# openshmem-org/openshmem-async

Hardware: AMD Instinct MI355X
Metric: GiB/s device-resident shmem_double_sum_to_all, nreduce=32Mi, 1/2/4/8 GPUs (higher is better)
Workload: dtype f64; 1 GPU; local reduce (fold acc = acc + in) of shmem_double_sum_to_all, 1 PE; nreduce=33554432, type=double, op=sum, PE_size=1, algo=fold, parallelism=one PE per GPU x1, transport=none (one PE: the step is the local fold, no exchange), arrays=symmetric heap (shmem_malloc, HBM)

## Files before the change

openshmem-async_amd/csrc/fold_kernels.hip:

```cpp
#include <hip/hip_ext.h>

#include <algorithm>
#include <atomic>
#include <mutex>
#include <vector>

#include "fold_ops.h"

namespace shmx {

enum KernelKind { kKindFold = 0, kKindCopy = 1, kKindPeers = 2, kKindGather = 3, kKindOrders = 4 };
namespace {
constexpr size_t kClockPairs = 4096;
struct KClock {
    std::mutex mu;
    std::atomic<bool> on{false};
    std::vector<hipEvent_t> ev;
    std::vector<int> kind;
    size_t used = 0;
    size_t dropped = 0;
} g_kclock;

bool clock_pair(int kind, hipEvent_t *a, hipEvent_t *b) {
    if (!g_kclock.on.load(std::memory_order_relaxed)) return false;
    std::lock_guard<std::mutex> lk(g_kclock.mu);
    if (g_kclock.used >= kClockPairs) {
        ++g_kclock.dropped;
        return false;
    }
    if (g_kclock.ev.size() < 2 * (g_kclock.used + 1)) {
// ... 67 lines not shown
    size_t nvec;
    size_t tail;
    int peers;
    unsigned long long *sig_word;
    unsigned long long sig_value;
    void *out2;
};

__device__ __forceinline__ void signal_host_done(const FoldArgs &args) {
    if (!args.sig_word) return;
    asm volatile("s_waitcnt vmcnt(0)" ::: "memory");
    __syncthreads();
    if (threadIdx.x == 0)
        __hip_atomic_store(args.sig_word, args.sig_value, __ATOMIC_RELEASE, __HIP_MEMORY_SCOPE_SYSTEM);
}


template <typename T, int OP, int NIN, int UNROLL, int NT>
__device__ __forceinline__ void fold_body(const FoldArgs &args) {
    constexpr int E = 16 / sizeof(T);
    const int nins = NIN > 0 ? NIN : args.nins;
    const size_t tid = (size_t)blockIdx.x * kBlock + threadIdx.x;
    const size_t nthr = (size_t)gridDim.x * kBlock;

    {
        T *out = static_cast<T *>(args.out);
        const size_t body_end = args.head + args.nvec * E;
        const size_t nscalar = args.head + args.tail;
        for (size_t s = tid; s < nscalar; s += nthr) {
            const size_t i = s < args.head ? s : body_end + (s - args.head);
            T acc = static_cast<const T *>(args.ins[0])[i];
            for (int k = 1; k < nins; ++k)
                acc = Op<T, OP>::ap(acc, static_cast<const T *>(args.ins[k])[i]);
            out[i] = acc;
            if constexpr (NIN == 1)
                if (args.out2) static_cast<T *>(args.out2)[i] = acc;
        }
    }
    if (args.nvec == 0) return;

    u32x4 *out = reinterpret_cast<u32x4 *>(static_cast<T *>(args.out) + args.head);
    u32x4 *out2 = NIN == 1 && args.out2 ? reinterpret_cast<u32x4 *>(static_cast<T *>(args.out2) + args.head)
                                        : nullptr;
    const size_t nvec = args.nvec;
    const size_t step = (size_t)gridDim.x * kBlock * UNROLL;
    for (size_t base = (size_t)blockIdx.x * kBlock * UNROLL; base < nvec;
// ... 31 lines not shown
                    u32x4 nxt[UNROLL];
#pragma unroll
                    for (int u = 0; u < UNROLL; ++u) nxt[u] = ld16<NT>(in_k(k) + v0 + u * kBlock);
#pragma unroll
                    for (int u = 0; u < UNROLL; ++u) {
                        acc[u] = apply16<T, OP>(acc[u], cur[u]);
                        cur[u] = nxt[u];
                    }
                }
#pragma unroll
                for (int u = 0; u < UNROLL; ++u) acc[u] = apply16<T, OP>(acc[u], cur[u]);
            } else {
                for (int k = 1; k < nins; ++k) {
                    const u32x4 *ink = reinterpret_cast<const u32x4 *>(
                        static_cast<const T *>(args.ins[k]) + args.head);
                    u32x4 x[UNROLL];
#pragma unroll
                    for (int u = 0; u < UNROLL; ++u) x[u] = ld16<NT>(ink + v0 + u * kBlock);
#pragma unroll
                    for (int u = 0; u < UNROLL; ++u) acc[u] = apply16<T, OP>(acc[u], x[u]);
                }
            }
#pragma unroll
            for (int u = 0; u < UNROLL; ++u) st16<NT>(out + v0 + u * kBlock, acc[u]);
            if constexpr (NIN == 1)
                if (out2)
#pragma unroll
                    for (int u = 0; u < UNROLL; ++u) st16<NT>(out2 + v0 + u * kBlock, acc[u]);
        } else {
            for (int u = 0; u < UNROLL; ++u) {
                const size_t v = v0 + (size_t)u * kBlock;
                if (v >= nvec) break;
                u32x4 acc = ld16<NT>(reinterpret_cast<const u32x4 *>(
                                         static_cast<const T *>(args.ins[0]) + args.head) + v);
                for (int k = 1; k < nins; ++k)
                    acc = apply16<T, OP>(acc, ld16<NT>(reinterpret_cast<const u32x4 *>(
                                                 static_cast<const T *>(args.ins[k]) + args.head) + v));
                st16<NT>(out + v, acc);
                if constexpr (NIN == 1)
                    if (out2) st16<NT>(out2 + v, acc);
            }
        }
    }
}

template <typename T, int OP, int NIN, int UNROLL, int NT>
__global__ __launch_bounds__(kBlock) void fold_kernel(FoldArgs args) {
    fold_body<T, OP, NIN, UNROLL, NT>(args);
    signal_host_done(args);
}

constexpr int kUnrollN = 4;
constexpr int kUnrollFold2 = 4;

constexpr int peers_unroll(int maxin) { return maxin <= 8 ? 4 : 2; }

template <typename T, int OP, int MAXIN, int NT>
__global__ __launch_bounds__(kBlock) void fold_peers_kernel(FoldArgs args) {
    constexpr int E = 16 / sizeof(T);
    constexpr int U = peers_unroll(MAXIN);
    const int nins = args.nins;
    const size_t tid = (size_t)blockIdx.x * kBlock + threadIdx.x;
    const size_t nthr = (size_t)gridDim.x * kBlock;
// ... 10 lines not shown
    }
    if (args.nvec == 0) return;
    auto in = [&](int k) {
        return reinterpret_cast<const u32x4 *>(static_cast<const T *>(args.ins[k]) + args.head);
    };
    u32x4 *out = reinterpret_cast<u32x4 *>(static_cast<T *>(args.out) + args.head);
    const size_t nvec = args.nvec;
    const size_t step = (size_t)gridDim.x * kBlock * U;
    for (size_t base = (size_t)blockIdx.x * kBlock * U; base < nvec; base += step) {
        const size_t v0 = base + threadIdx.x;
        if (base + (size_t)kBlock * U <= nvec) {
            u32x4 x[MAXIN][U];
#pragma unroll
            for (int k = 0; k < MAXIN; ++k)
                if (k < nins)
#pragma unroll
                    for (int u = 0; u < U; ++u) x[k][u] = ld16<NT>(in(k) + v0 + u * kBlock);
#pragma unroll
            for (int u = 0; u < U; ++u) {
                u32x4 acc = x[0][u];
#pragma unroll
                for (int k = 1; k < MAXIN; ++k)
                    if (k < nins) acc = apply16<T, OP>(acc, x[k][u]);
                st16<NT>(out + v0 + u * kBlock, acc);
            }
        } else {
            for (int u = 0; u < U; ++u) {
                const size_t v = v0 + (size_t)u * kBlock;
                if (v >= nvec) break;
                u32x4 acc = ld16<NT>(in(0) + v);
                for (int k = 1; k < nins; ++k) acc = apply16<T, OP>(acc, ld16<NT>(in(k) + v));
                st16<NT>(out + v, acc);
            }
        }
    }
}

constexpr int kUnrollOrders = 1;

struct OrdersArgs {
    void *outs[kMaxFoldInputs];
    const void *ins[kMaxFoldInputs];
    int nins;
    size_t head, nvec, tail;
};

template <typename T, int OP, int MAXIN, bool ROLLED, typename V, typename Ap, typename St>
__device__ __forceinline__ void fold_orders_of(const V (&x)[MAXIN], int nins, Ap ap, St store) {
    if constexpr (ROLLED) {
#pragma unroll 1
        for (int k = 0; k < nins; ++k) {
            V acc = x[0];
#pragma unroll
            for (int j = 1; j < MAXIN; ++j)
                if (j == k) acc = x[j];
// ... 29 lines not shown
        for (size_t s = tid; s < nscalar; s += nthr) {
            const size_t i = s < args.head ? s : body_end + (s - args.head);
            T x[MAXIN];
#pragma unroll
            for (int k = 0; k < MAXIN; ++k)
                if (k < nins) x[k] = static_cast<const T *>(args.ins[k])[i];
            fold_orders_of<T, OP, MAXIN, ROLLED>(
                x, nins, [](T a, T b) { return Op<T, OP>::ap(a, b); },
                [&](int k, T r) { static_cast<T *>(args.outs[k])[i] = r; });
        }
    }
    if (args.nvec == 0) return;
    auto in = [&](int k) {
        return reinterpret_cast<const u32x4 *>(static_cast<const T *>(args.ins[k]) + args.head);
    };
    auto out = [&](int k) { return reinterpret_cast<u32x4 *>(static_cast<T *>(args.outs[k]) + args.head); };
    auto ap16 = [](u32x4 a, u32x4 b) { return apply16<T, OP>(a, b); };
    const size_t nvec = args.nvec;
    for (size_t v = tid; v < nvec; v += nthr) {
        u32x4 x[MAXIN];
#pragma unroll
        for (int k = 0; k < MAXIN; ++k)
            if (k < nins) x[k] = ld16<NT>(in(k) + v);
        fold_orders_of<T, OP, MAXIN, ROLLED>(x, nins, ap16, [&](int k, u32x4 r) { st16<NT>(out(k) + v, r); });
    }
}


static size_t grid_for(const FoldArgs &a, int unroll) {
    size_t work_blocks;
    if (a.nvec > 0)
        work_blocks = (a.nvec + (size_t)kBlock * unroll - 1) / ((size_t)kBlock * unroll);
    else
        work_blocks = (a.head + a.tail + kBlock - 1) / kBlock;
    const size_t cap = a.nvec == 0 ? 2048 : (size_t)1 << 30;
    size_t blocks = work_blocks < cap ? work_blocks : cap;
    if (blocks < 1) blocks = 1;
    if (blocks > (size_t)INT_MAX) blocks = INT_MAX;
    return blocks;
}

hipError_t enqueue_marker(unsigned long long *word, unsigned long long value, hipStream_t stream) {
    return hipStreamWriteValue64(stream, word, value, 0);
}

template <typename T, int OP, int NT>
hipError_t launch_typed_grid(const FoldArgs &a, hipStream_t stream);
// ... 98 lines not shown
    case SHMEMX_OP_SUM: return launch_nt<T, SHMEMX_OP_SUM>(a, s);
    case SHMEMX_OP_PROD: return launch_nt<T, SHMEMX_OP_PROD>(a, s);
    default: return hipErrorInvalidValue;
    }
}

}

size_t type_size(int type) {
    switch (type) {
    case SHMEMX_TYPE_SHORT: return sizeof(short);
    case SHMEMX_TYPE_INT: return sizeof(int);
    case SHMEMX_TYPE_LONG: return sizeof(long);
    case SHMEMX_TYPE_LONGLONG: return sizeof(long long);
    case SHMEMX_TYPE_FLOAT: return sizeof(float);
    case SHMEMX_TYPE_DOUBLE: return sizeof(double);
    case SHMEMX_TYPE_LONGDOUBLE: return sizeof(long double);
    case SHMEMX_TYPE_COMPLEXD: return 2 * sizeof(double);
    case SHMEMX_TYPE_COMPLEXF: return 2 * sizeof(float);
    default: return 0;
    }
}

bool op_valid(int type, int op) {
    if (type < 0 || type >= SHMEMX_NTYPES || op < 0 || op >= SHMEMX_NOPS) return false;
    switch (op) {
    case SHMEMX_OP_SUM:
    case SHMEMX_OP_PROD: return true;
    case SHMEMX_OP_AND:
    case SHMEMX_OP_OR:
    case SHMEMX_OP_XOR: return type <= SHMEMX_TYPE_LONGLONG;
    default: return type != SHMEMX_TYPE_COMPLEXD && type != SHMEMX_TYPE_COMPLEXF;
    }
}

bool op_on_device(int type, int op) { return op_valid(type, op); }

namespace {

hipError_t dispatch(int type, int op, FoldArgs &a, const void *const *ptrs, int nptrs, size_t n,
                    hipStream_t stream) {
    const size_t sz = type_size(type);
    const uintptr_t off = reinterpret_cast<uintptr_t>(ptrs[0]) & 15u;
    bool same = (off % sz) == 0;
    for (int k = 1; k < nptrs && same; ++k)
        same = (reinterpret_cast<uintptr_t>(ptrs[k]) & 15u) == off;
    if (same) {
        size_t head = ((16 - off) & 15u) / sz;
        if (head > n) head = n;
        const size_t E = 16 / sz;
        a.head = head;
        a.nvec = (n - head) / E;
        a.tail = n - head - a.nvec * E;
    } else {
        a.head = n;
        a.nvec = 0;
        a.tail = 0;
    }
    if (a.nins == 1) {
        switch (sz) {
        case 2: return launch_copy<short>(a, stream);
        case 4: return launch_copy<int>(a, stream);
        case 8: return launch_copy<long>(a, stream);
        case 16: return launch_copy<cplxd>(a, stream);
        default: return hipErrorInvalidValue;
        }
    }
    switch (type) {
    case SHMEMX_TYPE_SHORT: return launch_int_ops<short>(op, a, stream);
    case SHMEMX_TYPE_INT: return launch_int_ops<int>(op, a, stream);
    case SHMEMX_TYPE_LONG:
    case SHMEMX_TYPE_LONGLONG: return launch_int_ops<long>(op, a, stream);
    case SHMEMX_TYPE_FLOAT: return launch_fp_ops<float>(op, a, stream);
    case SHMEMX_TYPE_DOUBLE: return launch_fp_ops<double>(op, a, stream);
    case SHMEMX_TYPE_LONGDOUBLE: return launch_fp_ops<ld80>(op, a, stream);
    case SHMEMX_TYPE_COMPLEXD: return launch_cplx_ops<cplxd>(op, a, stream);
    case SHMEMX_TYPE_COMPLEXF: return launch_cplx_ops<cplxf>(op, a, stream);
    default: return hipErrorInvalidValue;
    }
}

}

hipError_t launch_fold(int type, int op, void *out, const void *const *ins,
                       int nins, size_t n, hipStream_t stream) {
    if (!op_on_device(type, op) || nins < 1 || nins > kMaxFoldInputs || !out)
        return hipErrorInvalidValue;
    if (n == 0) return hipSuccess;
    FoldArgs a{};
    a.out = out;
    a.nins = nins;
    const void *ptrs[kMaxFoldInputs + 1];
    ptrs[0] = out;
    for (int k = 0; k < nins; ++k) {
        if (!ins[k]) return hipErrorInvalidValue;
        a.ins[k] = ins[k];
        ptrs[k + 1] = ins[k];
    }
    return dispatch(type, op, a, ptrs, nins + 1, n, stream);
}

bool copy_one_workgroup(int type, const void *dst, const void *src, size_t n) {
    const size_t sz = type_size(type);
    if (!sz || !n) return false;
    const uintptr_t off = reinterpret_cast<uintptr_t>(dst) & 15u;
    if (off % sz != 0 || (reinterpret_cast<uintptr_t>(src) & 15u) != off)
        return n <= (size_t)kBlock;
    size_t head = ((16 - off) & 15u) / sz;
    if (head > n) head = n;
    const size_t E = 16 / sz, nvec = (n - head) / E, tail = n - head - nvec * E;
    if (nvec == 0) return head + tail <= (size_t)kBlock;
    return nvec <= (size_t)kBlock * kUnrollCopy;
}

hipError_t launch_fold_signal(int type, int op, void *out, const void *const *ins, int nins, size_t n,
                              hipStream_t stream, const HostSignal &sig) {
    if (!op_on_device(type, op) || nins < 1 || nins > kMaxFoldInputs || !out || !sig.word)
        return hipErrorInvalidValue;
    if (n == 0) return launch_host_signal(sig, stream);
    FoldArgs a{};
    a.out = out;
    a.nins = nins;
    a.sig_word = sig.word;
    a.sig_value = sig.value;
    const void *ptrs[kMaxFoldInputs + 1];
    ptrs[0] = out;
    for (int k = 0; k < nins; ++k) {
        if (!ins[k]) return hipErrorInvalidValue;
        a.ins[k] = ins[k];
        ptrs[k + 1] = ins[k];
    }
    return dispatch(type, op, a, ptrs, nins + 1, n, stream);
}

hipError_t launch_copy2_signal(int type, void *out, void *out2, const void *in, size_t n, hipStream_t stream,
                               const HostSignal &sig) {
    if (!op_on_device(type, SHMEMX_OP_SUM) || !out || !out2 || !in || !sig.word) return hipErrorInvalidValue;
    if (n == 0) return launch_host_signal(sig, stream);
    FoldArgs a{};
    a.out = out;
    a.out2 = out2;
    a.nins = 1;
    a.ins[0] = in;
    a.sig_word = sig.word;
    a.sig_value = sig.value;
    const void *ptrs[3] = {out, out2, in};
    return dispatch(type, SHMEMX_OP_SUM, a, ptrs, 3, n, stream);
}

hipError_t launch_host_signal(const HostSignal &sig, hipStream_t stream) {
    if (!sig.word) return hipErrorInvalidValue;
    return enqueue_marker(sig.word, sig.value, stream);
}

hipError_t launch_fold_peers(int type, int op, void *out, const void *const *ins, int nins, size_t n,
                             hipStream_t stream) {
    if (!op_on_device(type, op) || nins < 1 || nins > kMaxFoldInputs || !out)
        return hipErrorInvalidValue;
    if (n == 0) return hipSuccess;
    FoldArgs a{};
    a.out = out;
    a.nins = nins;
    a.peers = 1;
    const void *ptrs[kMaxFoldInputs + 1];
    ptrs[0] = out;
    for (int k = 0; k < nins; ++k) {
        if (!ins[k]) return hipErrorInvalidValue;
        a.ins[k] = ins[k];
        ptrs[k + 1] = ins[k];
    }
    return dispatch(type, op, a, ptrs, nins + 1, n, stream);
}

namespace {

template <typename T, int OP, int MAXIN, int NT>
void launch_orders_grid(const OrdersArgs &a, hipStream_t stream) {
    FoldArgs g{};
    g.head = a.head;
    g.nvec = a.nvec;
    g.tail = a.tail;
    launch_k(kKindOrders, fold_orders_kernel<T, OP, MAXIN, NT>,
             dim3((unsigned)grid_for(g, kUnrollOrders)), dim3(kBlock), stream, a);
}

template <typename T, int OP>
hipError_t launch_orders_typed(const OrdersArgs &a, size_t n, hipStream_t stream) {
    const bool nt = (size_t)(2 * a.nins) * n * sizeof(T) >= kNtThresholdBytes;
    if (a.nins <= 8) {
        if (nt) launch_orders_grid<T, OP, 8, 3>(a, stream);
        else launch_orders_grid<T, OP, 8, 0>(a, stream);
    } else {
        if (nt) launch_orders_grid<T, OP, 16, 3>(a, stream);
        else launch_orders_grid<T, OP, 16, 0>(a, stream);
    }
    return hipGetLastError();
}

template <typename T>
hipError_t launch_orders_ops(int op, const OrdersArgs &a, size_t n, hipStream_t stream) {
    return op == SHMEMX_OP_MIN ? launch_orders_typed<T, SHMEMX_OP_MIN>(a, n, stream)
                               : launch_orders_typed<T, SHMEMX_OP_MAX>(a, n, stream);
}

}

hipError_t launch_fold_orders(int type, int op, void *const *outs, const void *const *ins, int nins, size_t n,
                              hipStream_t stream) {
    if ((op != SHMEMX_OP_MIN && op != SHMEMX_OP_MAX) || nins < 1 || nins > kMaxFoldInputs || !outs || !ins)
        return hipErrorInvalidValue;
    if (n == 0) return hipSuccess;
    const size_t sz = type_size(type);
    OrdersArgs a{};
    a.nins = nins;
    const uintptr_t off = reinterpret_cast<uintptr_t>(ins[0]) & 15u;
    bool same = sz && (off % sz) == 0;
    for (int k = 0; k < nins; ++k) {
        if (!ins[k] || !outs[k]) return hipErrorInvalidValue;
        a.ins[k] = ins[k];
        a.outs[k] = outs[k];
        same = same && (reinterpret_cast<uintptr_t>(ins[k]) & 15u) == off &&
               (reinterpret_cast<uintptr_t>(outs[k]) & 15u) == off;
    }
    if (same) {
        const size_t E = 16 / sz;
        a.head = std::min(n, ((16 - off) & 15u) / sz);
        a.nvec = (n - a.head) / E;
        a.tail = n - a.head - a.nvec * E;
    } else {
        a.head = n;
    }
    switch (type) {
    case SHMEMX_TYPE_FLOAT: return launch_orders_ops<float>(op, a, n, stream);
    case SHMEMX_TYPE_DOUBLE: return launch_orders_ops<double>(op, a, n, stream);
    case SHMEMX_TYPE_LONGDOUBLE: return launch_orders_ops<ld80>(op, a, n, stream);
    default: return hipErrorInvalidValue;
    }
}

namespace {

struct CopySeg {
    const unsigned char *src;
    unsigned char *dst;
    size_t bytes;
};
struct GatherArgs {
    CopySeg seg[kMaxFoldInputs];
    int nseg;
    unsigned run;
};

constexpr int kGatherUnroll = 8;
constexpr unsigned kGatherRun = 256;

__global__ __launch_bounds__(kBlock) void gather_kernel(GatherArgs a) {
    const unsigned r = blockIdx.x / a.run;
    const CopySeg sg = a.seg[r % a.nseg];
    const size_t bx = (size_t)(r / a.nseg) * a.run + blockIdx.x % a.run, nbx = gridDim.x / a.nseg;
    const size_t tid = bx * kBlock + threadIdx.x;
    const size_t nthr = nbx * kBlock;
    const uintptr_t d = reinterpret_cast<uintptr_t>(sg.dst);
    const uintptr_t s = reinterpret_cast<uintptr_t>(sg.src);
    size_t head = (16 - (d & 15)) & 15;
    if (head > sg.bytes) head = sg.bytes;
    if (((s + head) & 15) != 0) {
        for (size_t i = tid; i < sg.bytes; i += nthr) sg.dst[i] = sg.src[i];
        return;
    }
    const size_t nvec = (sg.bytes - head) / 16;
    const size_t tail0 = head + nvec * 16;
    if (tid < head) sg.dst[tid] = sg.src[tid];
    if (tid < sg.bytes - tail0) sg.dst[tail0 + tid] = sg.src[tail0 + tid];
    const u32x4 *in = reinterpret_cast<const u32x4 *>(sg.src + head);
    u32x4 *out = reinterpret_cast<u32x4 *>(sg.dst + head);
    const size_t step = nthr * kGatherUnroll;
    size_t v = bx * kBlock * kGatherUnroll + threadIdx.x;
    for (; v + (size_t)(kGatherUnroll - 1) * kBlock < nvec; v += step) {
        u32x4 x[kGatherUnroll];
#pragma unroll
        for (int u = 0; u < kGatherUnroll; ++u) x[u] = __builtin_nontemporal_load(in + v + u * kBlock);
#pragma unroll
        for (int u = 0; u < kGatherUnroll; ++u) __builtin_nontemporal_store(x[u], out + v + u * kBlock);
    }
    for (int u = 0; u < kGatherUnroll; ++u) {
        const size_t w = v + (size_t)u * kBlock;
        if (w < nvec) __builtin_nontemporal_store(__builtin_nontemporal_load(in + w), out + w);
    }
}

}

hipError_t launch_gather(const void *const *srcs, void *const *dsts, const size_t *bytes, int nseg,
                         hipStream_t stream) {
    if (nseg < 0 || nseg > kMaxFoldInputs) return hipErrorInvalidValue;
    GatherArgs a{};
    size_t most = 0;
    int k = 0;
    for (int i = 0; i < nseg; ++i) {
        if (!bytes[i]) continue;
        if (!srcs[i] || !dsts[i]) return hipErrorInvalidValue;
        a.seg[k++] = CopySeg{static_cast<const unsigned char *>(srcs[i]),
                             static_cast<unsigned char *>(dsts[i]), bytes[i]};
        most = bytes[i] > most ? bytes[i] : most;
    }
    if (!k) return hipSuccess;
    size_t bx = (most / 16 + (size_t)kBlock * kGatherUnroll - 1) / ((size_t)kBlock * kGatherUnroll);
    if (bx < 1) bx = 1;
    if (bx > 65536) bx = 65536;
    const size_t run = bx < kGatherRun ? bx : kGatherRun;
// ... 9 lines not shown
```

openshmem-async_amd/csrc/fold_ops.h:

```cpp
#pragma once

#include <hip/hip_runtime.h>

#include <climits>
#include <cstdint>
#include <cstdlib>
#include <type_traits>

#include "internal.h"
#include "ld80.h"
#include "shmem_reduce_mi355x.h"

namespace shmx {

namespace {

typedef unsigned int u32x4 __attribute__((ext_vector_type(4)));

struct cplxd { double re, im; };
struct cplxf { float re, im; };

template <typename T> struct Wide { using U = std::make_unsigned_t<T>; };
template <> struct Wide<short> { using U = unsigned int; };

// ... 82 lines not shown
#undef SHMX_FP_OPS

#define SHMX_CPLX_OPS(C, S)                                                    \
    template <> struct Op<C, SHMEMX_OP_SUM> {                                \
        __device__ static C ap(C a, C b) {                                   \
            return C{a.re + b.re, a.im + b.im}; } };                         \
    template <> struct Op<C, SHMEMX_OP_PROD> {                               \
        __device__ static C ap(C a, C b) {                                   \
            C r; cmul<S>(a.re, a.im, b.re, b.im, r.re, r.im); return r; } };
SHMX_CPLX_OPS(cplxd, double)
SHMX_CPLX_OPS(cplxf, float)
#undef SHMX_CPLX_OPS

using x87::ld80;
template <> struct Op<ld80, SHMEMX_OP_SUM> {
    __device__ static ld80 ap(ld80 a, ld80 b) { return x87::add(a, b); } };
template <> struct Op<ld80, SHMEMX_OP_PROD> {
    __device__ static ld80 ap(ld80 a, ld80 b) { return x87::mul(a, b); } };
template <> struct Op<ld80, SHMEMX_OP_MIN> {
    __device__ static ld80 ap(ld80 a, ld80 b) { return x87::less(a, b) ? a : b; } };
template <> struct Op<ld80, SHMEMX_OP_MAX> {
    __device__ static ld80 ap(ld80 a, ld80 b) { return x87::greater(a, b) ? a : b; } };

template <int NT>
__device__ __forceinline__ u32x4 ld16(const u32x4 *p) {
    if constexpr ((NT & 1) != 0) return __builtin_nontemporal_load(p);
    else return *p;
}
template <int NT>
__device__ __forceinline__ void st16(u32x4 *p, u32x4 v) {
    if constexpr ((NT & 2) != 0) __builtin_nontemporal_store(v, p);
    else *p = v;
}

template <typename T, int OP>
__device__ __forceinline__ u32x4 apply16(u32x4 a, u32x4 b) {
    constexpr int E = 16 / sizeof(T);
    union U { u32x4 v; T e[E]; };
    U x, y;
    x.v = a;
    y.v = b;
#pragma unroll
    for (int e = 0; e < E; ++e) x.e[e] = Op<T, OP>::ap(x.e[e], y.e[e]);
    return x.v;
}

constexpr int kBlock = 256;

template <typename T, int OP>
constexpr bool kHeavyOp = std::is_same<T, ld80>::value ||
                          ((std::is_same<T, cplxd>::value || std::is_same<T, cplxf>::value) &&
                           OP == SHMEMX_OP_PROD);

}

}
// ... 1 lines not shown
```

openshmem-async_amd/csrc/internal.h:

```cpp
#pragma once

#include <hip/hip_runtime.h>
#include <cstddef>
#include <cstdint>

namespace shmx {

constexpr int kMaxFoldInputs = 16;

size_t type_size(int type);
bool op_valid(int type, int op);
bool op_on_device(int type, int op);

hipError_t launch_fold(int type, int op, void *out, const void *const *ins,
                       int nins, size_t n, hipStream_t stream);

struct HostSignal {
    unsigned long long *word;
    unsigned long long value;
};
HostSignal next_host_signal();
void wait_host_signal(const HostSignal &sig, hipStream_t s);
hipError_t launch_fold_signal(int type, int op, void *out, const void *const *ins, int nins, size_t n,
                              hipStream_t stream, const HostSignal &sig);
bool copy_one_workgroup(int type, const void *dst, const void *src, size_t n);
hipError_t launch_copy2_signal(int type, void *out, void *out2, const void *in, size_t n, hipStream_t stream,
                               const HostSignal &sig);
hipError_t launch_host_signal(const HostSignal &sig, hipStream_t stream);

hipError_t launch_fold_peers(int type, int op, void *out, const void *const *ins, int nins, size_t n,
                             hipStream_t stream);

hipError_t launch_fold_orders(int type, int op, void *const *outs, const void *const *ins, int nins, size_t n,
// ... 15 lines not shown
    unsigned int *err;
    unsigned int *seen;
    int nxcc;
    unsigned long long *fence_stats;
};
hipError_t launch_signal(const SignalArgs &a, hipStream_t stream);

constexpr size_t kFusedTinyElems = 4 * 256;
struct SignalFoldArgs {
    SignalArgs sig;
    unsigned long long *host_word;
    unsigned long long host_value;
    unsigned int *gsync;
    void *out;
    const void *ins[kMaxFoldInputs];
    int nins;
    size_t n;
    int two_shot;
    size_t lo, hi;
    int nseg;
    const void *gsrc[kMaxFoldInputs];
    void *gdst[kMaxFoldInputs];
    size_t glen[kMaxFoldInputs];
};
hipError_t launch_signal_fold(int type, int op, const SignalFoldArgs &a, hipStream_t stream);

constexpr int kChecksumMaxBlocks = 4096;
hipError_t launch_checksum(int type, const void *ptr, size_t n, unsigned long long *out,
                           unsigned long long epoch, hipStream_t stream);

int kernel_timing(int on);
int kernel_times(double *us, int *kind, int max, unsigned long long *dropped);


}
```

openshmem-async_amd/csrc/signal_kernels.hip:

```cpp
#include "fold_ops.h"

namespace shmx {

namespace {

constexpr int kXccIdReg = 20 | (0 << 6) | ((4 - 1) << 11);

__global__ __launch_bounds__(64) void sys_fence_kernel(unsigned int *seen) {
    if (threadIdx.x == 0) {
        __builtin_amdgcn_fence(__ATOMIC_ACQ_REL, "");
        const unsigned int xcc = (unsigned int)__builtin_amdgcn_s_getreg(kXccIdReg) & 15u;
        __hip_atomic_store(seen + blockIdx.x, kFenceSeen | xcc, __ATOMIC_RELAXED,
                           __HIP_MEMORY_SCOPE_SYSTEM);
    }
}

__device__ __forceinline__ void check_fence(const SignalArgs &a) {
    const int lane = threadIdx.x;
    unsigned int rec = 0;
    if (a.seen && lane < kFenceBlocks) {
        rec = __hip_atomic_load(a.seen + lane, __ATOMIC_RELAXED, __HIP_MEMORY_SCOPE_SYSTEM);
        __hip_atomic_store(a.seen + lane, 0u, __ATOMIC_RELAXED, __HIP_MEMORY_SCOPE_SYSTEM);
    }
    if (!a.seen) return;
// ... 133 lines not shown
        if (threadIdx.x == 0) {
            peer_handshake(a.sig);
            if (a.host_word)
                __hip_atomic_store(a.host_word, a.host_value, __ATOMIC_RELEASE, __HIP_MEMORY_SCOPE_SYSTEM);
        }
        return;
    }
    const size_t tid = (size_t)blockIdx.x * kBlock + threadIdx.x, nthr = (size_t)gridDim.x * kBlock;
    for (size_t i = tid; i < a.n; i += nthr) out[i] = fold_elem<T, OP>(a, i);
    __syncthreads();
    if (threadIdx.x == 0 &&
        __hip_atomic_fetch_add(count, 1u, __ATOMIC_RELAXED, __HIP_MEMORY_SCOPE_AGENT) == gridDim.x - 1) {
        __hip_atomic_store(count, 0u, __ATOMIC_RELAXED, __HIP_MEMORY_SCOPE_AGENT);
        peer_handshake(a.sig);
    }
}

template <typename T, int OP, int MAXIN>
__device__ __forceinline__ void fold_vecs(const SignalFoldArgs &a, u32x4 *out, size_t nvec, size_t tid,
                                          size_t nthr) {
    constexpr int U = kMaxFoldInputs / MAXIN;
    const size_t step = nthr * U;
    auto in = [&](int k) {
        return reinterpret_cast<const u32x4 *>(static_cast<const T *>(a.ins[k]) + a.lo);
    };
    size_t v = (tid / kBlock) * kBlock * U + tid % kBlock;
    for (; v + (size_t)(U - 1) * kBlock < nvec; v += step) {
        u32x4 x[MAXIN][U];
#pragma unroll
        for (int k = 0; k < MAXIN; ++k)
            if (k < a.nins)
#pragma unroll
                for (int u = 0; u < U; ++u) x[k][u] = __builtin_nontemporal_load(in(k) + v + u * kBlock);
#pragma unroll
        for (int u = 0; u < U; ++u) {
            u32x4 acc = x[0][u];
#pragma unroll
            for (int k = 1; k < MAXIN; ++k)
                if (k < a.nins) acc = apply16<T, OP>(acc, x[k][u]);
            out[v + u * kBlock] = acc;
        }
    }
    for (int u = 0; u < U; ++u) {
        const size_t w = v + (size_t)u * kBlock;
        if (w >= nvec) break;
        u32x4 acc = __builtin_nontemporal_load(in(0) + w);
        for (int k = 1; k < a.nins; ++k) acc = apply16<T, OP>(acc, __builtin_nontemporal_load(in(k) + w));
        out[w] = acc;
    }
}

template <typename T, int OP>
__device__ __forceinline__ void fold_span(const SignalFoldArgs &a, size_t tid, size_t nthr) {
    constexpr int E = 16 / sizeof(T);
    const size_t lo = a.lo, n = a.hi - a.lo;
    T *const out = static_cast<T *>(a.out) + lo;
    bool vec = (reinterpret_cast<uintptr_t>(out) & 15) == 0;
    for (int k = 0; k < a.nins; ++k)
        vec &= (reinterpret_cast<uintptr_t>(static_cast<const T *>(a.ins[k]) + lo) & 15) == 0;
    const size_t nvec = vec ? n / E : 0;
    u32x4 *const vout = reinterpret_cast<u32x4 *>(out);
    if constexpr (kHeavyOp<T, OP>) {
        for (size_t v = tid; v < nvec; v += nthr) {
            u32x4 acc = __builtin_nontemporal_load(reinterpret_cast<const u32x4 *>(
                                                       static_cast<const T *>(a.ins[0]) + lo) + v);
            for (int k = 1; k < a.nins; ++k)
                acc = apply16<T, OP>(acc, __builtin_nontemporal_load(reinterpret_cast<const u32x4 *>(
                                                  static_cast<const T *>(a.ins[k]) + lo) + v));
            vout[v] = acc;
        }
    } else if (a.nins <= 4) {
        fold_vecs<T, OP, 4>(a, vout, nvec, tid, nthr);
    } else if (a.nins <= 8) {
        fold_vecs<T, OP, 8>(a, vout, nvec, tid, nthr);
    } else {
        fold_vecs<T, OP, 16>(a, vout, nvec, tid, nthr);
    }
    for (size_t i = nvec * E + tid; i < n; i += nthr) {
        T acc = static_cast<const T *>(a.ins[0])[lo + i];
        for (int k = 1; k < a.nins; ++k) acc = Op<T, OP>::ap(acc, static_cast<const T *>(a.ins[k])[lo + i]);
        out[i] = acc;
    }
}

template <int MAXSEG>
__device__ __forceinline__ void gather_vecs(const SignalFoldArgs &a, size_t nvec, size_t tid, size_t nthr) {
    constexpr int U = kMaxFoldInputs / MAXSEG;
    for (size_t v = (tid / kBlock) * kBlock * U + tid % kBlock; v < nvec; v += nthr * U) {
        u32x4 x[MAXSEG][U];
#pragma unroll
        for (int k = 0; k < MAXSEG; ++k)
#pragma unroll
            for (int u = 0; u < U; ++u)
                if (k < a.nseg && v + u * kBlock < a.glen[k] / 16)
                    x[k][u] = __builtin_nontemporal_load(static_cast<const u32x4 *>(a.gsrc[k]) + v + u * kBlock);
#pragma unroll
        for (int k = 0; k < MAXSEG; ++k)
#pragma unroll
            for (int u = 0; u < U; ++u)
                if (k < a.nseg && v + u * kBlock < a.glen[k] / 16)
                    static_cast<u32x4 *>(a.gdst[k])[v + u * kBlock] = x[k][u];
    }
}

__device__ __forceinline__ void gather_span(const SignalFoldArgs &a, size_t tid, size_t nthr) {
    bool vec = true;
    size_t most = 0;
    for (int k = 0; k < a.nseg; ++k) {
        vec &= ((reinterpret_cast<uintptr_t>(a.gsrc[k]) | reinterpret_cast<uintptr_t>(a.gdst[k])) & 15) == 0;
        most = a.glen[k] > most ? a.glen[k] : most;
    }
    if (!vec) {
        for (int k = 0; k < a.nseg; ++k)
            for (size_t i = tid; i < a.glen[k]; i += nthr)
                static_cast<unsigned char *>(a.gdst[k])[i] = static_cast<const unsigned char *>(a.gsrc[k])[i];
        return;
    }
    if (a.nseg <= 4) gather_vecs<4>(a, most / 16, tid, nthr);
    else if (a.nseg <= 8) gather_vecs<8>(a, most / 16, tid, nthr);
    else gather_vecs<16>(a, most / 16, tid, nthr);
    for (int k = 0; k < a.nseg; ++k)
        for (size_t i = a.glen[k] / 16 * 16 + tid; i < a.glen[k]; i += nthr)
            static_cast<unsigned char *>(a.gdst[k])[i] = static_cast<const unsigned char *>(a.gsrc[k])[i];
}

__device__ void grid_handshake(const SignalFoldArgs &a, unsigned int gen_now) {
    unsigned int *const count = a.gsync, *const gen = a.gsync + 1;
    __syncthreads();
    if (threadIdx.x == 0) {
        __builtin_amdgcn_fence(__ATOMIC_RELEASE, "");
        if (__hip_atomic_fetch_add(count, 1u, __ATOMIC_RELAXED, __HIP_MEMORY_SCOPE_AGENT) == gridDim.x - 1) {
            peer_handshake(a.sig);
            __hip_atomic_store(count, 0u, __ATOMIC_RELAXED, __HIP_MEMORY_SCOPE_AGENT);
            __hip_atomic_store(gen, gen_now + 1u, __ATOMIC_RELEASE, __HIP_MEMORY_SCOPE_AGENT);
        } else {
            const unsigned long long t0 = __builtin_amdgcn_s_memrealtime();
            while (__hip_atomic_load(gen, __ATOMIC_RELAXED, __HIP_MEMORY_SCOPE_AGENT) == gen_now) {
                if (__builtin_amdgcn_s_memrealtime() - t0 > a.sig.timeout_ticks) {
                    __hip_atomic_store(a.sig.err, 1u, __ATOMIC_RELAXED, __HIP_MEMORY_SCOPE_SYSTEM);
                    break;
                }
                __builtin_amdgcn_s_sleep(2);
            }
        }
        __builtin_amdgcn_fence(__ATOMIC_ACQUIRE, "");
    }
// ... 81 lines not shown
    case SHMEMX_OP_PROD: return sf_launch<T, SHMEMX_OP_PROD>(a, s);
    case SHMEMX_OP_AND:
        if constexpr (integral) return sf_launch<T, SHMEMX_OP_AND>(a, s);
        break;
    case SHMEMX_OP_OR:
        if constexpr (integral) return sf_launch<T, SHMEMX_OP_OR>(a, s);
        break;
    case SHMEMX_OP_XOR:
        if constexpr (integral) return sf_launch<T, SHMEMX_OP_XOR>(a, s);
        break;
    case SHMEMX_OP_MIN:
        if constexpr (!cplx) return sf_launch<T, SHMEMX_OP_MIN>(a, s);
        break;
    case SHMEMX_OP_MAX:
        if constexpr (!cplx) return sf_launch<T, SHMEMX_OP_MAX>(a, s);
        break;
    default: break;
    }
    return hipErrorInvalidValue;
}

}

hipError_t launch_signal_fold(int type, int op, const SignalFoldArgs &a, hipStream_t stream) {
    if (!op_on_device(type, op) || a.nins < 1 || a.nins > kMaxFoldInputs || !a.out || !a.gsync ||
        !a.sig.seen || !a.sig.fence_stats || a.sig.P < 1 || a.sig.P > kMaxFoldInputs || !a.sig.mine ||
        !a.sig.err)
        return hipErrorInvalidValue;
    for (int k = 0; k < a.nins; ++k)
        if (!a.ins[k]) return hipErrorInvalidValue;
    for (int i = 0; i < a.sig.P; ++i)
        if (a.sig.pe[i] != a.sig.me && !a.sig.peer[i]) return hipErrorInvalidValue;
    if (a.two_shot) {
        if (a.lo > a.hi || a.hi > a.n || a.nseg < 0 || a.nseg > kMaxFoldInputs) return hipErrorInvalidValue;
        for (int k = 0; k < a.nseg; ++k)
            if (a.glen[k] && (!a.gsrc[k] || !a.gdst[k])) return hipErrorInvalidValue;
    }
    switch (type) {
    case SHMEMX_TYPE_SHORT: return sf_ops<short>(op, a, stream);
    case SHMEMX_TYPE_INT: return sf_ops<int>(op, a, stream);
    case SHMEMX_TYPE_LONG:
    case SHMEMX_TYPE_LONGLONG: return sf_ops<long>(op, a, stream);
    case SHMEMX_TYPE_FLOAT: return sf_ops<float>(op, a, stream);
    case SHMEMX_TYPE_DOUBLE: return sf_ops<double>(op, a, stream);
    case SHMEMX_TYPE_LONGDOUBLE: return sf_ops<ld80>(op, a, stream);
    case SHMEMX_TYPE_COMPLEXD: return sf_ops<cplxd>(op, a, stream);
    case SHMEMX_TYPE_COMPLEXF: return sf_ops<cplxf>(op, a, stream);
    default: return hipErrorInvalidValue;
    }
}

hipError_t launch_signal(const SignalArgs &a, hipStream_t stream) {
    if (a.P < 1 || a.P > kMaxFoldInputs || !a.mine || !a.err) return hipErrorInvalidValue;
    for (int i = 0; i < a.P; ++i)
        if (a.pe[i] != a.me && !a.peer[i]) return hipErrorInvalidValue;
    hipLaunchKernelGGL(signal_kernel, dim3(1), dim3(64), 0, stream, a);
    return hipGetLastError();
}

hipError_t launch_sys_fence(hipStream_t stream, unsigned int *seen) {
// ... 7 lines not shown
```

Before: 2054 GiB/s.

## Vectorize folds and gathers when pointers are only element-aligned, not mutually 16B-aligned

Replaces the per-call-site alignment checks with a shared vec_split helper that keeps the 16-byte vector path whenever all pointers are element-aligned, aligning the head on the output pointer only. To support inputs whose 16-byte chunks are misaligned, ld16 and some st16 calls now use an under-aligned (2-byte) vector type. The signal fold and gather kernels gain head/body/tail splits so mismatched offsets no longer fall back to scalar or byte loops. The cost is that every vector load is now declared under-aligned, which may produce weaker load instructions on the common aligned path such as the one-PE shmalloc fold.

```diff
diff --git a/openshmem-async_amd/csrc/fold_kernels.hip b/openshmem-async_amd/csrc/fold_kernels.hip
--- a/openshmem-async_amd/csrc/fold_kernels.hip
+++ b/openshmem-async_amd/csrc/fold_kernels.hip
@@ -6,6 +6,7 @@
 #include <vector>
 
 #include "fold_ops.h"
+#include "vec_split.h"
 
 namespace shmx {
 
@@ -119,6 +120,7 @@
     const int nins = NIN > 0 ? NIN : args.nins;
     const size_t tid = (size_t)blockIdx.x * kBlock + threadIdx.x;
     const size_t nthr = (size_t)gridDim.x * kBlock;
+    constexpr bool OFF = NIN == 1 ? kCopyOutOff<T> : kOutOff<T>;
 
     {
         T *out = static_cast<T *>(args.out);
@@ -196,11 +198,11 @@
                 }
             }
 #pragma unroll
-            for (int u = 0; u < UNROLL; ++u) st16<NT>(out + v0 + u * kBlock, acc[u]);
+            for (int u = 0; u < UNROLL; ++u) st16<NT, OFF>(out + v0 + u * kBlock, acc[u]);
             if constexpr (NIN == 1)
                 if (out2)
 #pragma unroll
-                    for (int u = 0; u < UNROLL; ++u) st16<NT>(out2 + v0 + u * kBlock, acc[u]);
+                    for (int u = 0; u < UNROLL; ++u) st16<NT, true>(out2 + v0 + u * kBlock, acc[u]);
         } else {
             for (int u = 0; u < UNROLL; ++u) {
                 const size_t v = v0 + (size_t)u * kBlock;
@@ -210,9 +212,9 @@
                 for (int k = 1; k < nins; ++k)
                     acc = apply16<T, OP>(acc, ld16<NT>(reinterpret_cast<const u32x4 *>(
                                                  static_cast<const T *>(args.ins[k]) + args.head) + v));
-                st16<NT>(out + v, acc);
+                st16<NT, OFF>(out + v, acc);
                 if constexpr (NIN == 1)
-                    if (out2) st16<NT>(out2 + v, acc);
+                    if (out2) st16<NT, true>(out2 + v, acc);
             }
         }
     }
@@ -269,7 +271,7 @@
 #pragma unroll
                 for (int k = 1; k < MAXIN; ++k)
                     if (k < nins) acc = apply16<T, OP>(acc, x[k][u]);
-                st16<NT>(out + v0 + u * kBlock, acc);
+                st16<NT, kOutOff<T>>(out + v0 + u * kBlock, acc);
             }
         } else {
             for (int u = 0; u < U; ++u) {
@@ -277,7 +279,7 @@
                 if (v >= nvec) break;
                 u32x4 acc = ld16<NT>(in(0) + v);
                 for (int k = 1; k < nins; ++k) acc = apply16<T, OP>(acc, ld16<NT>(in(k) + v));
-                st16<NT>(out + v, acc);
+                st16<NT, kOutOff<T>>(out + v, acc);
             }
         }
     }
@@ -353,7 +355,10 @@
 #pragma unroll
         for (int k = 0; k < MAXIN; ++k)
             if (k < nins) x[k] = ld16<NT>(in(k) + v);
-        fold_orders_of<T, OP, MAXIN, ROLLED>(x, nins, ap16, [&](int k, u32x4 r) { st16<NT>(out(k) + v, r); });
+        fold_orders_of<T, OP, MAXIN, ROLLED>(x, nins, ap16, [&](int k, u32x4 r) {
+            if (kCAlign<T> == 16 || k == 0) st16<NT>(out(k) + v, r);
+            else st16<NT, true>(out(k) + v, r);
+        });
     }
 }
 
@@ -498,6 +503,14 @@
     }
 }
 
+size_t type_align(int type) {
+    switch (type) {
+    case SHMEMX_TYPE_COMPLEXD: return alignof(double);
+    case SHMEMX_TYPE_COMPLEXF: return alignof(float);
+    default: return type_size(type);
+    }
+}
+
 bool op_valid(int type, int op) {
     if (type < 0 || type >= SHMEMX_NTYPES || op < 0 || op >= SHMEMX_NOPS) return false;
     switch (op) {
@@ -514,25 +527,13 @@
 
 namespace {
 
-hipError_t dispatch(int type, int op, FoldArgs &a, const void *const *ptrs, int nptrs, size_t n,
+hipError_t dispatch(int type, int op, FoldArgs &a, const void *const *outs, int nouts, size_t n,
                     hipStream_t stream) {
     const size_t sz = type_size(type);
-    const uintptr_t off = reinterpret_cast<uintptr_t>(ptrs[0]) & 15u;
-    bool same = (off % sz) == 0;
-    for (int k = 1; k < nptrs && same; ++k)
-        same = (reinterpret_cast<uintptr_t>(ptrs[k]) & 15u) == off;
-    if (same) {
-        size_t head = ((16 - off) & 15u) / sz;
-        if (head > n) head = n;
-        const size_t E = 16 / sz;
-        a.head = head;
-        a.nvec = (n - head) / E;
-        a.tail = n - head - a.nvec * E;
-    } else {
-        a.head = n;
-        a.nvec = 0;
-        a.tail = 0;
-    }
+    const VecSplit sp = vec_split(outs, nouts, a.ins, a.nins, n, sz, type_align(type));
+    a.head = sp.head;
+    a.nvec = sp.nvec;
+    a.tail = sp.tail;
     if (a.nins == 1) {
         switch (sz) {
         case 2: return launch_copy<short>(a, stream);
@@ -566,27 +567,20 @@
     FoldArgs a{};
     a.out = out;
     a.nins = nins;
-    const void *ptrs[kMaxFoldInputs + 1];
-    ptrs[0] = out;
     for (int k = 0; k < nins; ++k) {
         if (!ins[k]) return hipErrorInvalidValue;
         a.ins[k] = ins[k];
-        ptrs[k + 1] = ins[k];
-    }
-    return dispatch(type, op, a, ptrs, nins + 1, n, stream);
+    }
+    const void *outs[1] = {out};
+    return dispatch(type, op, a, outs, 1, n, stream);
 }
 
 bool copy_one_workgroup(int type, const void *dst, const void *src, size_t n) {
     const size_t sz = type_size(type);
     if (!sz || !n) return false;
-    const uintptr_t off = reinterpret_cast<uintptr_t>(dst) & 15u;
-    if (off % sz != 0 || (reinterpret_cast<uintptr_t>(src) & 15u) != off)
-        return n <= (size_t)kBlock;
-    size_t head = ((16 - off) & 15u) / sz;
-    if (head > n) head = n;
-    const size_t E = 16 / sz, nvec = (n - head) / E, tail = n - head - nvec * E;
-    if (nvec == 0) return head + tail <= (size_t)kBlock;
-    return nvec <= (size_t)kBlock * kUnrollCopy;
+    const VecSplit sp = vec_split(&dst, 1, &src, 1, n, sz, type_align(type));
+    if (sp.nvec == 0) return sp.head + sp.tail <= (size_t)kBlock;
+    return sp.nvec <= (size_t)kBlock * kUnrollCopy;
 }
 
 hipError_t launch_fold_signal(int type, int op, void *out, const void *const *ins, int nins, size_t n,
@@ -599,14 +593,12 @@
     a.nins = nins;
     a.sig_word = sig.word;
     a.sig_value = sig.value;
-    const void *ptrs[kMaxFoldInputs + 1];
-    ptrs[0] = out;
     for (int k = 0; k < nins; ++k) {
         if (!ins[k]) return hipErrorInvalidValue;
         a.ins[k] = ins[k];
-        ptrs[k + 1] = ins[k];
-    }
-    return dispatch(type, op, a, ptrs, nins + 1, n, stream);
+    }
+    const void *outs[1] = {out};
+    return dispatch(type, op, a, outs, 1, n, stream);
 }
 
 hipError_t launch_copy2_signal(int type, void *out, void *out2, const void *in, size_t n, hipStream_t stream,
@@ -620,8 +612,8 @@
     a.ins[0] = in;
     a.sig_word = sig.word;
     a.sig_value = sig.value;
-    const void *ptrs[3] = {out, out2, in};
-    return dispatch(type, SHMEMX_OP_SUM, a, ptrs, 3, n, stream);
+    const void *outs[2] = {out, out2};
+    return dispatch(type, SHMEMX_OP_SUM, a, outs, 2, n, stream);
 }
 
 hipError_t launch_host_signal(const HostSignal &sig, hipStream_t stream) {
@@ -638,14 +630,12 @@
     a.out = out;
     a.nins = nins;
     a.peers = 1;
-    const void *ptrs[kMaxFoldInputs + 1];
-    ptrs[0] = out;
     for (int k = 0; k < nins; ++k) {
         if (!ins[k]) return hipErrorInvalidValue;
         a.ins[k] = ins[k];
-        ptrs[k + 1] = ins[k];
-    }
-    return dispatch(type, op, a, ptrs, nins + 1, n, stream);
+    }
+    const void *outs[1] = {out};
+    return dispatch(type, op, a, outs, 1, n, stream);
 }
 
 namespace {
@@ -689,23 +679,15 @@
     const size_t sz = type_size(type);
     OrdersArgs a{};
     a.nins = nins;
-    const uintptr_t off = reinterpret_cast<uintptr_t>(ins[0]) & 15u;
-    bool same = sz && (off % sz) == 0;
     for (int k = 0; k < nins; ++k) {
         if (!ins[k] || !outs[k]) return hipErrorInvalidValue;
         a.ins[k] = ins[k];
         a.outs[k] = outs[k];
-        same = same && (reinterpret_cast<uintptr_t>(ins[k]) & 15u) == off &&
-               (reinterpret_cast<uintptr_t>(outs[k]) & 15u) == off;
-    }
-    if (same) {
-        const size_t E = 16 / sz;
-        a.head = std::min(n, ((16 - off) & 15u) / sz);
-        a.nvec = (n - a.head) / E;
-        a.tail = n - a.head - a.nvec * E;
-    } else {
-        a.head = n;
-    }
+    }
+    const VecSplit sp = vec_split(a.outs, nins, a.ins, nins, n, sz, type_align(type));
+    a.head = sp.head;
+    a.nvec = sp.nvec;
+    a.tail = sp.tail;
     switch (type) {
     case SHMEMX_TYPE_FLOAT: return launch_orders_ops<float>(op, a, n, stream);
     case SHMEMX_TYPE_DOUBLE: return launch_orders_ops<double>(op, a, n, stream);
@@ -740,7 +722,7 @@
     const uintptr_t s = reinterpret_cast<uintptr_t>(sg.src);
     size_t head = (16 - (d & 15)) & 15;
     if (head > sg.bytes) head = sg.bytes;
-    if (((s + head) & 15) != 0) {
+    if (((s + head) & 3) != 0) {
         for (size_t i = tid; i < sg.bytes; i += nthr) sg.dst[i] = sg.src[i];
         return;
     }
@@ -755,13 +737,13 @@
     for (; v + (size_t)(kGatherUnroll - 1) * kBlock < nvec; v += step) {
         u32x4 x[kGatherUnroll];
 #pragma unroll
-        for (int u = 0; u < kGatherUnroll; ++u) x[u] = __builtin_nontemporal_load(in + v + u * kBlock);
+        for (int u = 0; u < kGatherUnroll; ++u) x[u] = ld16<1>(in + v + u * kBlock);
 #pragma unroll
         for (int u = 0; u < kGatherUnroll; ++u) __builtin_nontemporal_store(x[u], out + v + u * kBlock);
     }
     for (int u = 0; u < kGatherUnroll; ++u) {
         const size_t w = v + (size_t)u * kBlock;
-        if (w < nvec) __builtin_nontemporal_store(__builtin_nontemporal_load(in + w), out + w);
+        if (w < nvec) __builtin_nontemporal_store(ld16<1>(in + w), out + w);
     }
 }
 
diff --git a/openshmem-async_amd/csrc/fold_ops.h b/openshmem-async_amd/csrc/fold_ops.h
--- a/openshmem-async_amd/csrc/fold_ops.h
+++ b/openshmem-async_amd/csrc/fold_ops.h
@@ -128,16 +128,31 @@
 template <> struct Op<ld80, SHMEMX_OP_MAX> {
     __device__ static ld80 ap(ld80 a, ld80 b) { return x87::greater(a, b) ? a : b; } };
 
+typedef u32x4 u32x4_off __attribute__((aligned(2)));
+
 template <int NT>
 __device__ __forceinline__ u32x4 ld16(const u32x4 *p) {
-    if constexpr ((NT & 1) != 0) return __builtin_nontemporal_load(p);
-    else return *p;
+    const u32x4_off *q = reinterpret_cast<const u32x4_off *>(p);
+    if constexpr ((NT & 1) != 0) return __builtin_nontemporal_load(q);
+    else return *q;
 }
-template <int NT>
+template <int NT, bool OFF = false>
 __device__ __forceinline__ void st16(u32x4 *p, u32x4 v) {
-    if constexpr ((NT & 2) != 0) __builtin_nontemporal_store(v, p);
-    else *p = v;
+    if constexpr (OFF) {
+        u32x4_off *q = reinterpret_cast<u32x4_off *>(p);
+        if constexpr ((NT & 2) != 0) __builtin_nontemporal_store(v, q);
+        else *q = v;
+    } else {
+        if constexpr ((NT & 2) != 0) __builtin_nontemporal_store(v, p);
+        else *p = v;
+    }
 }
+
+template <typename T> constexpr size_t kCAlign = sizeof(T);
+template <> constexpr size_t kCAlign<cplxd> = 8;
+template <> constexpr size_t kCAlign<cplxf> = 4;
+template <typename T> constexpr bool kOutOff = kCAlign<T> < sizeof(T);
+template <typename T> constexpr bool kCopyOutOff = sizeof(T) >= 8;
 
 template <typename T, int OP>
 __device__ __forceinline__ u32x4 apply16(u32x4 a, u32x4 b) {
diff --git a/openshmem-async_amd/csrc/internal.h b/openshmem-async_amd/csrc/internal.h
--- a/openshmem-async_amd/csrc/internal.h
+++ b/openshmem-async_amd/csrc/internal.h
@@ -9,6 +9,7 @@
 constexpr int kMaxFoldInputs = 16;
 
 size_t type_size(int type);
+size_t type_align(int type);
 bool op_valid(int type, int op);
 bool op_on_device(int type, int op);
 
@@ -70,6 +71,7 @@
     const void *gsrc[kMaxFoldInputs];
     void *gdst[kMaxFoldInputs];
     size_t glen[kMaxFoldInputs];
+    size_t fold_head, fold_nvec;
 };
 hipError_t launch_signal_fold(int type, int op, const SignalFoldArgs &a, hipStream_t stream);
 
diff --git a/openshmem-async_amd/csrc/signal_kernels.hip b/openshmem-async_amd/csrc/signal_kernels.hip
--- a/openshmem-async_amd/csrc/signal_kernels.hip
+++ b/openshmem-async_amd/csrc/signal_kernels.hip
@@ -1,4 +1,5 @@
 #include "fold_ops.h"
+#include "vec_split.h"
 
 namespace shmx {
 
@@ -179,7 +180,7 @@
     constexpr int U = kMaxFoldInputs / MAXIN;
     const size_t step = nthr * U;
     auto in = [&](int k) {
-        return reinterpret_cast<const u32x4 *>(static_cast<const T *>(a.ins[k]) + a.lo);
+        return reinterpret_cast<const u32x4 *>(static_cast<const T *>(a.ins[k]) + a.lo + a.fold_head);
     };
     size_t v = (tid / kBlock) * kBlock * U + tid % kBlock;
     for (; v + (size_t)(U - 1) * kBlock < nvec; v += step) {
@@ -188,43 +189,38 @@
         for (int k = 0; k < MAXIN; ++k)
             if (k < a.nins)
 #pragma unroll
-                for (int u = 0; u < U; ++u) x[k][u] = __builtin_nontemporal_load(in(k) + v + u * kBlock);
+                for (int u = 0; u < U; ++u) x[k][u] = ld16<1>(in(k) + v + u * kBlock);
 #pragma unroll
         for (int u = 0; u < U; ++u) {
             u32x4 acc = x[0][u];
 #pragma unroll
             for (int k = 1; k < MAXIN; ++k)
                 if (k < a.nins) acc = apply16<T, OP>(acc, x[k][u]);
-            out[v + u * kBlock] = acc;
+            st16<0, kOutOff<T>>(out + v + u * kBlock, acc);
         }
     }
     for (int u = 0; u < U; ++u) {
         const size_t w = v + (size_t)u * kBlock;
         if (w >= nvec) break;
-        u32x4 acc = __builtin_nontemporal_load(in(0) + w);
-        for (int k = 1; k < a.nins; ++k) acc = apply16<T, OP>(acc, __builtin_nontemporal_load(in(k) + w));
-        out[w] = acc;
+        u32x4 acc = ld16<1>(in(0) + w);
+        for (int k = 1; k < a.nins; ++k) acc = apply16<T, OP>(acc, ld16<1>(in(k) + w));
+        st16<0, kOutOff<T>>(out + w, acc);
     }
 }
 
 template <typename T, int OP>
 __device__ __forceinline__ void fold_span(const SignalFoldArgs &a, size_t tid, size_t nthr) {
     constexpr int E = 16 / sizeof(T);
-    const size_t lo = a.lo, n = a.hi - a.lo;
+    const size_t lo = a.lo, n = a.hi - a.lo, head = a.fold_head, nvec = a.fold_nvec;
     T *const out = static_cast<T *>(a.out) + lo;
-    bool vec = (reinterpret_cast<uintptr_t>(out) & 15) == 0;
-    for (int k = 0; k < a.nins; ++k)
-        vec &= (reinterpret_cast<uintptr_t>(static_cast<const T *>(a.ins[k]) + lo) & 15) == 0;
-    const size_t nvec = vec ? n / E : 0;
-    u32x4 *const vout = reinterpret_cast<u32x4 *>(out);
+    u32x4 *const vout = reinterpret_cast<u32x4 *>(out + head);
     if constexpr (kHeavyOp<T, OP>) {
         for (size_t v = tid; v < nvec; v += nthr) {
-            u32x4 acc = __builtin_nontemporal_load(reinterpret_cast<const u32x4 *>(
-                                                       static_cast<const T *>(a.ins[0]) + lo) + v);
+            u32x4 acc = ld16<1>(reinterpret_cast<const u32x4 *>(static_cast<const T *>(a.ins[0]) + lo + head) + v);
             for (int k = 1; k < a.nins; ++k)
-                acc = apply16<T, OP>(acc, __builtin_nontemporal_load(reinterpret_cast<const u32x4 *>(
-                                                  static_cast<const T *>(a.ins[k]) + lo) + v));
-            vout[v] = acc;
+                acc = apply16<T, OP>(acc, ld16<1>(reinterpret_cast<const u32x4 *>(
+                                              static_cast<const T *>(a.ins[k]) + lo + head) + v));
+            st16<0, kOutOff<T>>(vout + v, acc);
         }
     } else if (a.nins <= 4) {
         fold_vecs<T, OP, 4>(a, vout, nvec, tid, nthr);
@@ -233,11 +229,24 @@
     } else {
         fold_vecs<T, OP, 16>(a, vout, nvec, tid, nthr);
     }
-    for (size_t i = nvec * E + tid; i < n; i += nthr) {
+    const size_t body_end = head + nvec * E, nscalar = n - nvec * E;
+    for (size_t s = tid; s < nscalar; s += nthr) {
+        const size_t i = s < head ? s : body_end + (s - head);
         T acc = static_cast<const T *>(a.ins[0])[lo + i];
         for (int k = 1; k < a.nins; ++k) acc = Op<T, OP>::ap(acc, static_cast<const T *>(a.ins[k])[lo + i]);
         out[i] = acc;
     }
+}
+
+struct SegSplit {
+    size_t head, nvec;
+};
+__device__ __forceinline__ SegSplit seg_split(const SignalFoldArgs &a, int k) {
+    const uintptr_t d = reinterpret_cast<uintptr_t>(a.gdst[k]), s = reinterpret_cast<uintptr_t>(a.gsrc[k]);
+    size_t head = (16 - (d & 15)) & 15;
+    if (head > a.glen[k]) head = a.glen[k];
+    if (((s + head) & 3) != 0) return SegSplit{0, 0};
+    return SegSplit{head, (a.glen[k] - head) / 16};
 }
 
 template <int MAXSEG>
@@ -246,39 +255,44 @@
     for (size_t v = (tid / kBlock) * kBlock * U + tid % kBlock; v < nvec; v += nthr * U) {
         u32x4 x[MAXSEG][U];
 #pragma unroll
-        for (int k = 0; k < MAXSEG; ++k)
+        for (int k = 0; k < MAXSEG; ++k) {
+            if (k >= a.nseg) continue;
+            const SegSplit sp = seg_split(a, k);
+            const u32x4 *src =
+                reinterpret_cast<const u32x4 *>(static_cast<const unsigned char *>(a.gsrc[k]) + sp.head);
 #pragma unroll
             for (int u = 0; u < U; ++u)
-                if (k < a.nseg && v + u * kBlock < a.glen[k] / 16)
-                    x[k][u] = __builtin_nontemporal_load(static_cast<const u32x4 *>(a.gsrc[k]) + v + u * kBlock);
-#pragma unroll
-        for (int k = 0; k < MAXSEG; ++k)
+                if (v + u * kBlock < sp.nvec) x[k][u] = ld16<1>(src + v + u * kBlock);
+        }
+#pragma unroll
+        for (int k = 0; k < MAXSEG; ++k) {
+            if (k >= a.nseg) continue;
+            const SegSplit sp = seg_split(a, k);
+            u32x4 *dst = reinterpret_cast<u32x4 *>(static_cast<unsigned char *>(a.gdst[k]) + sp.head);
 #pragma unroll
             for (int u = 0; u < U; ++u)
-                if (k < a.nseg && v + u * kBlock < a.glen[k] / 16)
-                    static_cast<u32x4 *>(a.gdst[k])[v + u * kBlock] = x[k][u];
+                if (v + u * kBlock < sp.nvec) dst[v + u * kBlock] = x[k][u];
+        }
     }
 }
 
 __device__ __forceinline__ void gather_span(const SignalFoldArgs &a, size_t tid, size_t nthr) {
-    bool vec = true;
     size_t most = 0;
     for (int k = 0; k < a.nseg; ++k) {
-        vec &= ((reinterpret_cast<uintptr_t>(a.gsrc[k]) | reinterpret_cast<uintptr_t>(a.gdst[k])) & 15) == 0;
-        most = a.glen[k] > most ? a.glen[k] : most;
-    }
-    if (!vec) {
-        for (int k = 0; k < a.nseg; ++k)
-            for (size_t i = tid; i < a.glen[k]; i += nthr)
-                static_cast<unsigned char *>(a.gdst[k])[i] = static_cast<const unsigned char *>(a.gsrc[k])[i];
-        return;
-    }
-    if (a.nseg <= 4) gather_vecs<4>(a, most / 16, tid, nthr);
-    else if (a.nseg <= 8) gather_vecs<8>(a, most / 16, tid, nthr);
-    else gather_vecs<16>(a, most / 16, tid, nthr);
-    for (int k = 0; k < a.nseg; ++k)
-        for (size_t i = a.glen[k] / 16 * 16 + tid; i < a.glen[k]; i += nthr)
+        const size_t nv = seg_split(a, k).nvec;
+        most = nv > most ? nv : most;
+    }
+    if (a.nseg <= 4) gather_vecs<4>(a, most, tid, nthr);
+    else if (a.nseg <= 8) gather_vecs<8>(a, most, tid, nthr);
+    else gather_vecs<16>(a, most, tid, nthr);
+    for (int k = 0; k < a.nseg; ++k) {
+        const SegSplit sp = seg_split(a, k);
+        const size_t body_end = sp.head + sp.nvec * 16, nbytes = a.glen[k] - sp.nvec * 16;
+        for (size_t b = tid; b < nbytes; b += nthr) {
+            const size_t i = b < sp.head ? b : body_end + (b - sp.head);
             static_cast<unsigned char *>(a.gdst[k])[i] = static_cast<const unsigned char *>(a.gsrc[k])[i];
+        }
+    }
 }
 
 __device__ void grid_handshake(const SignalFoldArgs &a, unsigned int gen_now) {
@@ -406,7 +420,8 @@
 
 }
 
-hipError_t launch_signal_fold(int type, int op, const SignalFoldArgs &a, hipStream_t stream) {
+hipError_t launch_signal_fold(int type, int op, const SignalFoldArgs &a0, hipStream_t stream) {
+    SignalFoldArgs a = a0;
     if (!op_on_device(type, op) || a.nins < 1 || a.nins > kMaxFoldInputs || !a.out || !a.gsync ||
         !a.sig.seen || !a.sig.fence_stats || a.sig.P < 1 || a.sig.P > kMaxFoldInputs || !a.sig.mine ||
         !a.sig.err)
@@ -420,6 +435,16 @@
         for (int k = 0; k < a.nseg; ++k)
             if (a.glen[k] && (!a.gsrc[k] || !a.gdst[k])) return hipErrorInvalidValue;
     }
+    a.fold_head = a.fold_nvec = 0;
+    if (a.two_shot) {
+        const size_t sz = type_size(type);
+        const void *out = static_cast<const unsigned char *>(a.out) + a.lo * sz;
+        const void *ins[kMaxFoldInputs];
+        for (int k = 0; k < a.nins; ++k) ins[k] = static_cast<const unsigned char *>(a.ins[k]) + a.lo * sz;
+        const VecSplit sp = vec_split(&out, 1, ins, a.nins, a.hi - a.lo, sz, type_align(type));
+        a.fold_head = sp.nvec ? sp.head : 0;
+        a.fold_nvec = sp.nvec;
+    }
     switch (type) {
     case SHMEMX_TYPE_SHORT: return sf_ops<short>(op, a, stream);
     case SHMEMX_TYPE_INT: return sf_ops<int>(op, a, stream);
diff --git a/openshmem-async_amd/csrc/vec_split.h b/openshmem-async_amd/csrc/vec_split.h
--- /dev/null
+++ b/openshmem-async_amd/csrc/vec_split.h
@@ -0,0 +1,41 @@
+#pragma once
+
+#include <cstddef>
+#include <cstdint>
+
+namespace shmx {
+
+struct VecSplit {
+    size_t head = 0;
+    size_t nvec = 0;
+    size_t tail = 0;
+    bool off16 = false;
+};
+
+inline VecSplit vec_split(const void *const *outs, int nouts, const void *const *ins, int nins, size_t n,
+                          size_t sz, size_t calign) {
+    VecSplit s;
+    bool ok = (sz == 2 || sz == 4 || sz == 8 || sz == 16) && nouts >= 1 &&
+              (calign == 2 || calign == 4 || calign == 8 || calign == 16) && calign <= sz;
+    for (int k = 0; k < nouts && ok; ++k) ok = reinterpret_cast<uintptr_t>(outs[k]) % calign == 0;
+    for (int k = 0; k < nins && ok; ++k) ok = reinterpret_cast<uintptr_t>(ins[k]) % calign == 0;
+    if (!ok) {
+        s.head = n;
+        return s;
+    }
+    const size_t off = reinterpret_cast<uintptr_t>(outs[0]) & 15u;
+    size_t head = off % sz == 0 ? ((16 - off) & 15u) / sz : 0;
+    if (head > n) head = n;
+    const size_t E = 16 / sz;
+    s.head = head;
+    s.nvec = (n - head) / E;
+    s.tail = n - head - s.nvec * E;
+    if (s.nvec) {
+        const uintptr_t skip = head * sz;
+        for (int k = 0; k < nouts; ++k) s.off16 |= ((reinterpret_cast<uintptr_t>(outs[k]) + skip) & 15u) != 0;
+        for (int k = 0; k < nins; ++k) s.off16 |= ((reinterpret_cast<uintptr_t>(ins[k]) + skip) & 15u) != 0;
+    }
+    return s;
+}
+
+}
```

Result: no change. 2057 GiB/s (median of 6 runs) (+0.2%).
